# xh92117/Retinex-image-Enhancement

Hardware: AMD Instinct MI355X
Metric: images/sec at 512x512 bs=32 per GPU (UP-Retinex forward) (higher is better)
Workload: dtype f32; 1 GPU; configs[1]: bs=32/GPU 512x512 plain forward, fp32; global_batch=32, image_size=512, variant=plain, parallelism=batch-shard x1 (no data-path collective)

## Files before the change

include/upr.h:

```cpp
#ifndef UPR_H_
#define UPR_H_

#include <stddef.h>
#include <stdint.h>

#ifdef __cplusplus
extern "C" {
#endif

enum { UPR_F32 = 0, UPR_F16 = 1, UPR_F32_SPLIT = 2, UPR_F32_SPLIT_REGS = 3 };

enum {
  UPR_OK = 0,
  UPR_ERR_ARG = -1,
  UPR_ERR_SHAPE = -2,
  UPR_ERR_MISSING_PARAM = -3,
  UPR_ERR_WORKSPACE = -4,
  UPR_ERR_UNSUPPORTED = -5
};

enum { UPR_MODEL_IENET_ONLY = 1, UPR_MODEL_HEAD_ONLY = 2 };

typedef struct UprModel UprModel;

// ... 43 lines not shown
int upr_retinex_decompose_bwd(const void* x, const void* illu, const void* g, void* gx, void* gillu, int B, int C,
                              int H, int W, int illu_c, int dtype, void* stream);

int upr_conv2d_nhwc(const void* x, int B, int H, int W, int Cin, const void* w, const float* bias, int Cout, int kh,
                    int kw, int stride, int pad, int dil, const void* residual, int relu, void* y, int dtype,
                    void* stream);

int upr_conv2d_nhwc_regs(const void* x, int B, int H, int W, int Cin, const void* w, const float* bias, int Cout,
                         int kh, int kw, int stride, int pad, int dil, const void* residual, int relu, void* y,
                         unsigned* overflow, void* stream);

int upr_split_f32(const float* x, void* y, size_t npix, int C, unsigned* overflow, void* stream);
int upr_unsplit_f32(const void* x, float* y, size_t npix, int C, void* stream);
size_t upr_pack_split_f32(const float* w, int Cout, int Cin, int kh, int kw, void* out, size_t out_bytes);

size_t upr_pack_split_w_f32(const float* w, int Cout, int Cin, int kh, int kw, const float* w2, int C2, void* out,
                            size_t out_bytes);
int upr_conv2d_nhwc_wsplit(const void* x, int B, int H, int W, int Cin, const void* blob, size_t blob_bytes,
                           const float* bias, int Cout, int kh, int kw, int stride, int pad, int dil,
                           const void* residual, int relu, void* y, const void* x2, int H2, int W2, int C2,
                           int stride2, unsigned* overflow, void* stream);
int upr_conv_wsplit_ran(void);

int upr_quantize_u8(const void* x, uint8_t* out, size_t n, int dtype, void* stream);

int upr_letterbox(const void* src, int src_kind, int H, int W, int top, int left, int nh, int nw, int Ho, int Wo,
                  const int32_t* xtab, const int32_t* ytab, int color, void* out, int out_kind, void* stream);

int upr_to_u8_hwc(const void* x, int C, int H, int W, int dtype, uint8_t* out, void* stream);

int upr_rgb2lab_u8(const uint8_t* rgb, uint8_t* lab, size_t npix, void* stream);
int upr_lab2rgb_u8(const uint8_t* lab, uint8_t* rgb, size_t npix, void* stream);

int upr_clahe_u8(const uint8_t* src, uint8_t* dst, uint8_t* lut_ws, int B, int H, int W, float clip, int tiles_x,
                 int tiles_y, void* stream);

size_t upr_clahe_enhance_workspace(int B, int H, int W, int tiles_x, int tiles_y);
int upr_clahe_enhance(const void* enh, void* out, void* workspace, int B, int H, int W, float clip, int tiles_x,
                      int tiles_y, int dtype, void* stream);

int upr_gray_hist(const void* x, int32_t* hist, int B, int H, int W, int dtype, void* stream);

int upr_multiscale(const void* x, const void* enh, void* out, double* sums, double* factor, int B, int H, int W,
                   int dtype, void* stream);

int upr_multiscale_features(const void* x, void* out, int B, int H, int W, int scale_idx, int dtype, void* stream);
// ... 51 lines not shown
```

retinex-image-enhancement_amd/csrc/conv_t2.hip:

```cpp
#include <algorithm>
#include <cstdlib>
#include <cstring>

#include "upr_common.h"

namespace upr {

typedef _Float16 t2h8 __attribute__((ext_vector_type(8)));
typedef _Float16 t2h4 __attribute__((ext_vector_type(4)));
typedef float t2f4 __attribute__((ext_vector_type(4)));

template <int KC, int COUT>
struct ConvT2Cfg {
  static constexpr int N = 4 * COUT;
  static constexpr int NSPLIT = N / 128;
  static constexpr int KS = KC / 32;
  static constexpr int NT = 8;
  static constexpr int TEAMS = 4 / NSPLIT;
  static constexpr int QPW = COUT >= 128 ? 1 : 128 / COUT;
  static constexpr int ROWS = QPW >= 2 ? QPW / 2 : 1;
  static constexpr int XS = QPW >= 2 ? 32 : 16;
  static constexpr int RSTR = COUT + 8;
  static constexpr int LDSW = ROWS * XS * RSTR * 2;
  static constexpr int OCC = KC >= 256 ? 1 : 2;
// ... 153 lines not shown
    __builtin_amdgcn_fence(__ATOMIC_RELEASE, "wavefront");
    __builtin_amdgcn_wave_barrier();
    __builtin_amdgcn_fence(__ATOMIC_ACQUIRE, "wavefront");
    const int b = g / (H * gpr), rem = g - b * H * gpr, y = rem / gpr, xg = (rem - y * gpr) * 16;
    const int q0 = ns * K::QPW, dy0 = q0 >> 1;
    constexpr int CPP = COUT / 4;
    constexpr int CHUNKS = K::ROWS * K::XS * CPP;
#pragma unroll
    for (int i = 0; i < CHUNKS / 64; ++i) {
      const int c = i * 64 + lane;
      const int row = c / (K::XS * CPP), xs = (c / CPP) % K::XS, part = c % CPP;
      const int xo = K::QPW >= 2 ? 2 * xg + xs : 2 * (xg + xs) + (q0 & 1);
      const f4 v = *(const f4*)(st + ((row * K::XS + xs) * RSTR + part * 4) * 4);
      float* dst = (float*)op.out + ((size_t)(b * 2 * H + 2 * y + dy0 + row) * (2 * W) + xo) * op.out_cs +
                   op.out_coff + part * 4;
      *(f4*)dst = v;
    }
    __builtin_amdgcn_wave_barrier();
#pragma unroll
    for (int q = 0; q < KQ; ++q) x0[q] = x1[q];
  }
}

template <int KC, int COUT>
static int launch_t2_f32(const ConvOp& op, hipStream_t st) {
  static int occ = 0;
  if (!occ) {
    if (hipOccupancyMaxActiveBlocksPerMultiprocessor(&occ, (const void*)conv_t2_f32_kernel<KC, COUT>, 256, 0) !=
            hipSuccess ||
        occ < 1)
      occ = 1;
  }
  int cus = 256;
  {
    int dev = 0;
    if (hipGetDevice(&dev) == hipSuccess) (void)hipDeviceGetAttribute(&cus, hipDeviceAttributeMultiprocessorCount, dev);
  }
  const int ngroups = op.B * op.Ho * (op.Wo / 16);
  const int teams = ConvT2Cfg<KC, COUT>::TEAMS;
  int grid = std::min(cus * occ, (ngroups + teams - 1) / teams);
  if (grid < 1) grid = 1;
  hipLaunchKernelGGL((conv_t2_f32_kernel<KC, COUT>), dim3(grid), dim3(256), 0, st, op, ngroups);
  return (int)hipGetLastError();
}

template <int KC, int COUT>
// ... 44 lines not shown
```

retinex-image-enhancement_amd/csrc/model.hip:

```cpp
#include <algorithm>
#include <atomic>
#include <cmath>
#include <cstdio>
#include <cstdlib>
#include <cstring>
#include <map>
#include <memory>
#include <mutex>
#include <string>
#include <vector>

#include "upr_common.h"
#include "../../include/upr.h"

namespace upr {

int launch_prep(const void* x, void* x2p, void* x3p, int B, int H, int W, int dtype, hipStream_t st);
int launch_preact_f16(const void* x, const float* sc, const float* sh, void* o, size_t npix, int C, hipStream_t st);
int launch_conv3(const void* x, const float* w, const float* bias, void* out0, void* out1, int B, int h, int wd,
                 int dtype, hipStream_t st, void* out2 = nullptr, const float* ps = nullptr,
                 const float* ph = nullptr);
int launch_fam_ca(const float* pool, const float* w1, const float* b1, const float* w2, const float* b2, float* ca,
                  int B, int HW, hipStream_t st);
int launch_fam_mix(const void* y, const float* ca, const float* P, float* mm, float* p, int B, int HW, int dtype,
// ... 202 lines not shown
static bool pack_split_w(int N, int K, const float* w, SplitWPack& out) {
  if (!w || N <= 0 || N % 64 || K <= 0 || K % 32) return false;
  out.W.assign((size_t)N * K * 2, (_Float16)0.f);
  out.scale.assign(N, 1.f);
  for (int n = 0; n < N; ++n) {
    const float* row = w + (size_t)n * K;
    float mx = 0.f;
    for (int k = 0; k < K; ++k) mx = std::max(mx, std::fabs(row[k]));
    const int sh = split_row_shift(mx);
    const float s = std::ldexp(1.f, sh);
    out.scale[n] = std::ldexp(1.f, -sh);
    _Float16* dst = out.W.data() + (size_t)n * K * 2;
    for (int k = 0; k < K; ++k) {
      const float ws = row[k] * s;
      const _Float16 hi = (_Float16)ws;
      _Float16* step = dst + (size_t)(k / 32) * 64;
      step[wsplit_kslot(k % 32)] = hi;
      step[32 + wsplit_kslot(k % 32)] = (_Float16)(ws - (float)hi);
    }
  }
  return true;
}

static std::vector<double> conv_w(const HostTensor& t, const std::vector<double>* mul) {
  std::vector<double> w = t.v;
  if (mul) {
    const size_t per = w.size() / mul->size();
    for (size_t n = 0; n < mul->size(); ++n)
      for (size_t i = 0; i < per; ++i) w[n * per + i] *= (*mul)[n];
  }
  return w;
}

static std::vector<double> compose(const std::vector<double>& A, int O, int Mdim, const std::vector<double>& W,
                                   int C, int khw) {
  std::vector<double> out((size_t)O * C * khw, 0.0);
  for (int o = 0; o < O; ++o)
    for (int m = 0; m < Mdim; ++m) {
      const double a = A[(size_t)o * Mdim + m];
      if (a == 0.0) continue;
      for (int i = 0; i < C * khw; ++i) out[(size_t)o * C * khw + i] += a * W[(size_t)m * C * khw + i];
    }
  return out;
}

static std::vector<double> cols(const std::vector<double>& A, int rows, int ncols, int c0, int n) {
// ... 30 lines not shown
};

static std::vector<double> conv3_kmajor(const std::vector<double>& w) {
  const size_t nout = w.size() / 27;
  std::vector<double> t(w.size());
  for (size_t o = 0; o < nout; ++o)
    for (size_t k = 0; k < 27; ++k) t[k * nout + o] = w[o * 27 + k];
  return t;
}

enum OpKind { OP_GEMM, OP_CONV3, OP_PREP, OP_FAM_CA, OP_FAM_MIX, OP_FAM_SA, OP_ASPP_G, OP_TAIL, OP_PREACT, OP_SPLIT };

struct Op {
  OpKind kind;
  std::string name;
  int layer = -1;
  int level = 0;
  int out = -1, out_cs = 0, out_coff = 0;
  int res1 = -1, res1_cs = 0, res2 = -1, res2_cs = 0;
  int relu = 0, store = kStoreNHWC;
  int pool_slot = -1;
  int split_layer = -1, split_exit = 0;
  size_t w64_w = SIZE_MAX, w64_scale = 0;
  int img_bias = 0;
  size_t head_w = 0; float head_b = 0.f;
  int in = -1, out1 = -1, out2 = -1;
  size_t ps = 0, ph = 0;
  size_t w = 0, b = 0;
  int fam = 0;
  size_t ca_w1 = 0, ca_b1 = 0, ca_w2 = 0, ca_b2 = 0, P = 0, sa_w = 0;
  float sa_b = 0.f;
  int lvl_shift = 0;
  size_t cst = 0;
};

}

struct UprModel {
  int dtype = 0;
  int use_preact = 0, use_aspp = 0, flags = 0;
  void* dev_blob = nullptr;
  size_t blob_bytes = 0;
  std::vector<upr::GemmLayer> layers;
  std::vector<upr::Op> ops;
  bool prof = false;
  std::vector<std::vector<hipEvent_t>> ev_pending;
// ... 5 lines not shown
  struct Side {
    hipStream_t s = nullptr;
    hipEvent_t fork = nullptr, join = nullptr;
    unsigned long long last_use = 0;
    ~Side() {
      if (s) (void)hipStreamSynchronize(s);
      if (join) (void)hipEventDestroy(join);
      if (fork) (void)hipEventDestroy(fork);
      if (s) (void)hipStreamDestroy(s);
    }
  };
  static constexpr size_t kMaxSides = 16;
  std::map<std::pair<int, hipStream_t>, std::shared_ptr<Side>> sides;
  unsigned long long side_clock = 0;
  std::mutex sides_mu;
  std::atomic<long long> forks{0};
  std::atomic<int> split_state{0};
  unsigned* ovf_dev = nullptr;
  volatile unsigned* ovf_host = nullptr;
  int split_regs = 0;
  int ring_split = 0;
  int split_w64 = 0;
  int w64_tile = 0;
  std::vector<int> op_forms;
  std::mutex forms_mu;
};

namespace upr {

struct BufGeom {
  int C;
  int shift;
  int is_f32;
  int pyramid;
};

static BufGeom buf_geom(int id, int use_aspp) {
  switch (id) {
    case B_X2P: return {3, 2, 0, 1};
    case B_X3P: return {3, 4, 0, 2};
    case B_X1: case B_S1IN: return {32, 0, 0, 0};
    case B_S2IN: return {32, 2, 0, 1};
    case B_S3IN: return {32, 4, 0, 2};
    case B_E1T: case B_X2: return {64, 1, 0, 0};
    case B_E2T: case B_X3: return {128, 2, 0, 0};
    case B_E3T: case B_X4: case B_B0T: case B_B0: case B_AP: case B_B1T: case B_X5: return {256, 3, 0, 0};
// ... 102 lines not shown
      o->split_layer = (int)m->layers.size() - 1;
      o->split_exit = i + 1 == names.size();
    }
    return true;
  }
  void make_w64(const std::vector<std::string>& names) {
    if (dt != kF32) return;
    for (const std::string& name : names)
      for (auto& o : m->ops) {
        if (o.kind != OP_GEMM || o.name != name) continue;
        const GemmLayer& L = m->layers[o.layer];
        bool fits = L.N % 64 == 0 && o.store == kStoreNHWC && o.pool_slot < 0 && !o.img_bias && o.out2 < 0 &&
                    !L.segs.empty() && L.segs.size() <= 2;
        int K = 0;
        for (const SegSpec& s : L.segs) {
          fits = fits && s.pre == kPreNone && s.C % 32 == 0 && s.kbase == K;
          K += s.kh * s.kw * s.C;
        }
        SplitWPack sp;
        if (!fits || K != L.Kpad || !pack_split_w(L.N, K, (const float*)(blob.bytes.data() + L.w), sp)) continue;
        o.w64_w = blob.add(sp.W.data(), sp.W.size() * 2);
        o.w64_scale = blob.add(sp.scale.data(), sp.scale.size() * 4);
      }
  }
  void gemm(const std::string& name, int layer, int level, int out, int out_cs, int relu, int res1 = -1,
            int res1_cs = 0, int res2 = -1, int res2_cs = 0, int store = kStoreNHWC, int out_coff = 0,
            int pool_slot = -1, int img_bias = 0) {
    Op o;
    o.kind = OP_GEMM; o.name = name; o.layer = layer; o.level = level; o.out = out; o.out_cs = out_cs; o.out_coff = out_coff;
    o.relu = relu; o.res1 = res1; o.res1_cs = res1_cs; o.res2 = res2; o.res2_cs = res2_cs; o.store = store;
    o.pool_slot = pool_slot; o.img_bias = img_bias;
    m->ops.push_back(o);
  }

  void block(const std::string& p, int in, int tmp, int out, int cin, int cout, int stride, int in_level,
             int pool_slot = -1) {
    const int lvl = in_level + (stride == 2 ? 1 : 0);
    const bool proj = stride != 1 || cin != cout;
    const HostTensor* w1 = T(p + ".conv1.weight");
    const HostTensor* w2 = T(p + ".conv2.weight");
    if (!ok) return;
    if (!m->use_preact) {
      BNFold bn1, bn2, bns;
      if (!bn_fold(P, p + ".bn1", cout, bn1) || !bn_fold(P, p + ".bn2", cout, bn2)) { ok = false; return; }
      std::vector<SegWeights> s1(1);
      s1[0].spec = seg(in, cin, cin, 0, 3, stride, 1, 1);
// ... 260 lines not shown
    bd.block(ie + ".bottleneck.0", B_X4, B_B0T, B_B0, 256, 256, 1, 3, 3);
    bd.aspp(ie + ".bottleneck.1", B_B0, B_AP);
    bd.block(ie + ".bottleneck.2", B_AP, B_B1T, B_X5, 256, 256, 1, 3);
  } else {
    bd.block(ie + ".bottleneck.0", B_X4, B_B0T, B_B0, 256, 256, 1, 3);
    bd.block(ie + ".bottleneck.1", B_B0, B_B1T, B_X5, 256, 256, 1, 3);
  }
  if (!bd.ok) return P.missing.empty() ? kErrShape : kErrMissingParam;
  bd.upblock(ie + ".dec3", B_X5, B_U3, B_V3, B_D3, 256, 128, 3, B_X3);
  if (m->split_state.load() == 1) {
    std::vector<std::string> region;
    for (const char* n : {".enc2.conv1", ".enc2.conv2", ".enc3.conv1", ".enc3.conv2", ".bottleneck.0.conv1",
                          ".bottleneck.0.conv2", ".bottleneck.1.conv1", ".bottleneck.1.conv2", ".dec3.up",
                          ".dec3.conv.0", ".dec3.conv.3"})
      region.push_back(ie + n);
    if (!bd.ok || !bd.make_split(region)) {
      for (auto& o : m->ops) o.split_layer = -1;
      m->split_state.store(0);
    }
    bd.kept.clear();
  }
  bd.upblock(ie + ".dec2", B_D3, B_U2, B_V2, B_D2, 128, 64, 2, B_X2);
  bd.upblock(ie + ".dec1", B_D2, B_U1, B_V1, B_D1, 64, 32, 1, B_X1);
  if (bd.ok && m->split_state.load() == 1 && m->split_regs && m->split_w64)
    bd.make_w64({ie + ".enc1.conv1", ie + ".enc1.conv2", ie + ".dec2.conv.0", ie + ".dec2.conv.3"});
  {
    const HostTensor* w0 = bd.T(ie + ".residual_head.0.weight");
    const HostTensor* b0 = bd.T(ie + ".residual_head.0.bias");
    const HostTensor* w2 = bd.T(ie + ".residual_head.2.weight");
    const HostTensor* b2 = bd.T(ie + ".residual_head.2.bias");
    if (!bd.ok) return kErrMissingParam;
    std::vector<SegWeights> s(1);
    s[0].spec = seg(B_D1, 32, 32, 0, 3, 1, 1, 1);
    s[0].w = w0->v;
    int l = bd.add_layer(32, s, b0->v);
    Op o;
    o.kind = OP_GEMM; o.name = ie + ".residual_head"; o.layer = l; o.level = 0; o.store = kStoreHeadIllu;
    o.head_w = blob.add_f32(w2->v); o.head_b = (float)b2->v[0];
    m->ops.push_back(o);
  }
  }
  if (!(m->flags & UPR_MODEL_IENET_ONLY)) {
    const HostTensor* wfu = bd.T("fusion.weight");
    const HostTensor* bfu = bd.T("fusion.bias");
    const HostTensor* wo = bd.T("output_layer.weight");
    const HostTensor* bo = bd.T("output_layer.bias");
// ... 86 lines not shown
  float* pool = (float*)buf(B_POOL);
  float* ca = (float*)buf(B_CA);
  float* ib = (float*)buf(B_IB);
  UPR_CHECK_HIP(hipMemsetAsync(pool, 0, (size_t)4 * B * 256 * 4 * kPoolEntryFloats, st));
  const int H4 = (H / 2) / 2, W4 = (W / 2) / 2, H16 = (H / 4) / 4, W16 = (W / 4) / 4;
  auto lvl_dims = [&](int lshift, int& h, int& w) {
    if (lshift == 2) { h = H4; w = W4; }
    else if (lshift == 4) { h = H16; w = W16; }
    else { h = H >> lshift; w = W >> lshift; }
  };
  float* illu32 = dt == kF16 ? (float*)buf(B_ILLU32) : (float*)illu;
  const size_t nops = m->ops.size();
  std::vector<hipEvent_t> evs;
  if (m->prof) {
    evs.resize(2 * nops);
    for (auto& e : evs) {
      if (!m->ev_free.empty()) { e = m->ev_free.back(); m->ev_free.pop_back(); }
      else UPR_CHECK_HIP(hipEventCreate(&e));
    }
    m->cur_flops.assign(nops, 0.0);
    m->cur_bytes.assign(nops, 0.0);
  }
  const double elt = dt == kF16 ? 2.0 : 4.0;
  auto split_op = [&](const Op& o, int ho, int wo) {
    const GemmLayer& L = m->layers[o.split_layer];
    ConvOp c;
    memset(&c, 0, sizeof(c));
    c.nseg = (int)L.segs.size();
    for (int i = 0; i < c.nseg; ++i) {
      const SegSpec& s = L.segs[i];
      ConvSeg& cs = c.seg[i];
      cs.src = buf(s.src);
      cs.C = s.C; cs.cs = s.cs; cs.coff = s.coff;
      cs.Hin = ho * s.stride; cs.Win = wo * s.stride;
      cs.kh = s.kh; cs.kw = s.kw; cs.stride = s.stride; cs.pad = s.pad; cs.dil = s.dil;
      cs.pre = kPreNone; cs.kbase = s.kbase;
    }
    c.B = B; c.Ho = ho; c.Wo = wo; c.N = L.N; c.Kpad = L.Kpad;
    c.W = blob + L.w;
    c.scale = fptr(L.scale);
    c.bias = L.bias != SIZE_MAX ? fptr(L.bias) : nullptr;
    c.res1 = o.res1 >= 0 ? buf(o.res1) : nullptr; c.res1_cs = 2 * o.res1_cs;
    c.res2 = o.res2 >= 0 ? buf(o.res2) : nullptr; c.res2_cs = 2 * o.res2_cs;
    c.split_res = c.res1 || c.res2;
    c.relu = o.relu;
    c.store = o.store;
    if (o.split_exit) { c.out_f32 = (float*)buf(o.out); c.out_f32_cs = o.out_cs; }
    else { c.split_out = buf(o.out); c.split_cs = 2 * o.out_cs; c.split_lo = o.out_cs; }
    c.ovf = m->ovf_dev;
    return c;
  };
  bool split_now = false;
  if (m->split_state.load() == 1) {
    int one = 1;
    if (m->ovf_host && *m->ovf_host) {
      if (m->split_state.compare_exchange_strong(one, 2))
        fprintf(stderr, "upr: an fp32 activation left the fp16 range; this model now runs its exact fp32 plan "
                      "(UPR_FP32_SPLIT=0 selects it from the start)\n");
    } else {
      split_now = true;
      for (const Op& o : m->ops)
        if (o.kind == OP_GEMM && o.split_layer >= 0) {
          int ho, wo;
          lvl_dims(o.level, ho, wo);
          if (launch_conv_wide(split_op(o, ho, wo), st, true) != kOk) split_now = false;
        }
    }
  }
  const bool regs_now = m->split_regs && m->ovf_dev && m->split_state.load() == 1 && !(m->ovf_host && *m->ovf_host);
  std::vector<int> forms(nops, 0);
  auto run_op = [&](size_t oi, hipStream_t st) -> int {
    const Op& o = m->ops[oi];
    int rc = kOk;
    if (m->prof) UPR_CHECK_HIP(hipEventRecord(evs[2 * oi], st));
    switch (o.kind) {
      case OP_PREP:
        rc = launch_prep(x, buf(B_X2P), buf(B_X3P), B, H, W, dt, st);
        break;
      case OP_CONV3: {
        int h, w;
        lvl_dims(o.lvl_shift, h, w);
        rc = launch_conv3(buf(o.in), fptr(o.w), fptr(o.b), buf(o.out), o.out1 >= 0 ? buf(o.out1) : nullptr, B, h, w,
                          dt, st, o.out2 >= 0 ? buf(o.out2) : nullptr, o.out2 >= 0 ? fptr(o.ps) : nullptr,
                          o.out2 >= 0 ? fptr(o.ph) : nullptr);
        break;
      }
      case OP_GEMM: {
        const GemmLayer& L = m->layers[o.layer];
        ConvOp c;
// ... 16 lines not shown
        }
        c.B = B; c.Ho = ho; c.Wo = wo; c.N = L.N; c.Kpad = L.Kpad;
        c.W = blob + L.w;
        c.scale = nullptr;
        c.bias = L.bias != SIZE_MAX ? fptr(L.bias) : nullptr;
        c.img_bias = o.img_bias ? ib : nullptr;
        c.res1 = o.res1 >= 0 ? buf(o.res1) : nullptr; c.res1_cs = o.res1_cs;
        c.relu = o.relu;
        c.res2 = o.res2 >= 0 ? buf(o.res2) : nullptr; c.res2_cs = o.res2_cs;
        c.store = o.store;
        if (o.store == kStoreHeadIllu) {
          c.head_w = fptr(o.head_w); c.head_b = o.head_b;
          c.x_nchw = (const float*)x; c.x_f16 = dt == kF16;
          c.illu = illu32; c.illu_f16 = 0;
          c.out = nullptr;
        } else {
          c.out = buf(o.out); c.out_cs = o.out_cs; c.out_coff = o.out_coff;
        }
        c.pool = o.pool_slot >= 0 ? pool + (size_t)o.pool_slot * B * 256 * kPoolEntryFloats : nullptr;
        if (o.out2 >= 0) {
          c.out2 = buf(o.out2); c.out2_cs = L.N;
          c.pre2_scale = fptr(o.ps); c.pre2_shift = fptr(o.ph);
        }
        if (split_now && o.split_layer >= 0) {
          rc = launch_conv_wide(split_op(o, ho, wo), st);
          forms[oi] = 1;
        } else {
          rc = kErrUnsupported;
          if (regs_now && dt == kF32 && o.w64_w != SIZE_MAX) {
            ConvOp cw = c;
            cw.W = blob + o.w64_w; cw.scale = fptr(o.w64_scale);
            cw.mma16 = 3; cw.ovf = m->ovf_dev;
            cw.ring_split = m->ring_split; cw.w64_tile = m->w64_tile;
            rc = launch_conv_wsplit(cw, st);
            if (rc == kOk) forms[oi] = 3;
          }
          if (rc == kErrUnsupported) {
            if (regs_now && dt == kF32) { c.mma16 = 1; c.ovf = m->ovf_dev; c.ring_split = m->ring_split; }
            rc = launch_conv(c, dt, st);
            forms[oi] = conv_last_form();
          }
        }
        if (m->prof) {
          const double Mpx = (double)B * ho * wo;
          double K = 0, bytes = (double)L.N * L.Kpad * elt;
          for (int i = 0; i < c.nseg; ++i) {
            K += (double)c.seg[i].kh * c.seg[i].kw * c.seg[i].C;
            bytes += (double)B * c.seg[i].Hin * c.seg[i].Win * c.seg[i].C * elt;
          }
          const double nout = o.store == kStoreHeadIllu ? 1.0 : (double)L.N;
// ... 210 lines not shown
  if ((flags & ~kKnownFlags) || (flags & kKnownFlags) == kKnownFlags) return UPR_ERR_ARG;
  ParamSet P;
  for (int i = 0; i < n_params; ++i) {
    const UprTensorDesc& d = params[i];
    if (!d.name || d.ndim < 0 || d.ndim > 4) return UPR_ERR_ARG;
    HostTensor t;
    int64_t n = 1;
    for (int k = 0; k < d.ndim; ++k) { t.shape.push_back(d.shape[k]); n *= d.shape[k]; }
    if (n > 0 && !d.data) return UPR_ERR_ARG;
    t.v.assign(d.data, d.data + n);
    P.t[d.name] = std::move(t);
  }
  std::unique_ptr<UprModel> m(new UprModel());
  m->dtype = dtype; m->use_preact = use_preact ? 1 : 0; m->use_aspp = use_aspp ? 1 : 0; m->flags = flags;
  const char* se = getenv("UPR_FP32_SPLIT");
  const bool split_env = !(se && *se && atoi(se) == 0);
  if (split_env && dtype == UPR_F32 && !m->use_preact && !m->use_aspp) m->split_state.store(1);
  const char* sr = getenv("UPR_FP32_SPLIT_REGS");
  m->split_regs = !(sr && *sr && atoi(sr) == 0);
  m->ring_split = ring_split_env();
  const char* sw = getenv("UPR_FP32_SPLIT_W64");
  m->split_w64 = !(sw && *sw && atoi(sw) == 0);
  m->w64_tile = w64_tile_env();
  int rc = build_model(m.get(), P);
  if (rc == kOk && m->split_state.load() == 1) {
    hipError_t e = hipMalloc((void**)&m->ovf_dev, 256);
    if (e == hipSuccess) e = hipMemset(m->ovf_dev, 0, 256);
    if (e == hipSuccess) e = hipHostMalloc((void**)&m->ovf_host, sizeof(unsigned), hipHostMallocDefault);
    if (e == hipSuccess) *m->ovf_host = 0u;
    else rc = (int)e;
  }
  if (rc != kOk) {
    if (m->dev_blob) (void)hipFree(m->dev_blob);
    if (m->ovf_dev) (void)hipFree(m->ovf_dev);
    if (m->ovf_host) (void)hipHostFree((void*)m->ovf_host);
    return rc;
  }
  *out = m.release();
  return UPR_OK;
}

size_t upr_model_workspace(const UprModel* model, int B, int H, int W) {
  if (!model || B <= 0 || H <= 0 || W <= 0) return 0;
  return ws_layout(model, B, H, W, nullptr);
}

// ... 226 lines not shown
  memset(&c, 0, sizeof(c));
  c.nseg = x2 ? 2 : 1;
  ConvSeg& s = c.seg[0];
  s.src = x; s.C = Cin; s.cs = Cin; s.coff = 0; s.Hin = H; s.Win = W;
  s.kh = kh; s.kw = kw; s.stride = stride; s.pad = pad; s.dil = dil; s.pre = kPreNone; s.kbase = 0;
  if (x2) {
    ConvSeg& t = c.seg[1];
    t.src = x2; t.C = C2; t.cs = C2; t.coff = 0; t.Hin = H2; t.Win = W2;
    t.kh = 1; t.kw = 1; t.stride = stride2; t.pad = 0; t.dil = 1; t.pre = kPreNone; t.kbase = K1;
  }
  c.B = B; c.Ho = Ho; c.Wo = Wo; c.N = Cout; c.Kpad = K;
  c.W = blob; c.scale = (const float*)((const uint8_t*)blob + soff);
  c.bias = bias; c.relu = relu;
  c.res2 = residual; c.res2_cs = Cout;
  c.out = y; c.out_cs = Cout; c.out_coff = 0; c.store = kStoreNHWC;
  c.mma16 = 3; c.ovf = overflow;
  c.ring_split = ring_split_env();
  c.w64_tile = w64_tile_env();
  return launch_conv_wsplit(c, (hipStream_t)stream);
}

int upr_conv_wsplit_ran(void) { return conv_last_wsplit_kernel(); }

int upr_split_f32(const float* x, void* y, size_t npix, int C, unsigned* overflow, void* stream) {
  if (!x || !y) return UPR_ERR_ARG;
  return launch_split_f32(x, y, npix, C, overflow, (hipStream_t)stream);
}

int upr_unsplit_f32(const void* x, float* y, size_t npix, int C, void* stream) {
  if (!x || !y) return UPR_ERR_ARG;
  return launch_unsplit_f32(x, y, npix, C, (hipStream_t)stream);
}

}
```

retinex-image-enhancement_amd/csrc/upr_common.h:

```cpp
#pragma once
#include <hip/hip_runtime.h>
#include <stdint.h>
#include <stddef.h>

#define UPR_CHECK_HIP(expr)                                  \
  do {                                                       \
    hipError_t _e = (expr);                                  \
    if (_e != hipSuccess) return (int)_e;                    \
  } while (0)

namespace upr {

typedef _Float16 half_t;

enum : int {
  kOk = 0,
  kErrArg = -1,
  kErrShape = -2,
  kErrMissingParam = -3,
  kErrWorkspace = -4,
  kErrUnsupported = -5,
};

enum DType : int { kF32 = 0, kF16 = 1 };
// ... 94 lines not shown
  return sh;
}

int launch_split_f32(const float* x, void* y, size_t npix, int C, unsigned* ovf, hipStream_t st);
int launch_unsplit_f32(const void* x, float* y, size_t npix, int C, hipStream_t st);

int launch_conv_out32(const ConvOp& op, hipStream_t stream);
int launch_conv_s2dg(const ConvOp& op, hipStream_t stream, bool probe = false);
int launch_conv_pw(const ConvOp& op, hipStream_t stream, bool probe = false);

int launch_conv(const ConvOp& op, int dtype, hipStream_t stream);
int conv_last_form();
void conv_set_last_form(int form);
int launch_conv_regs(const ConvOp& op, hipStream_t stream);

int launch_conv_ring32(const ConvOp& op, hipStream_t st);
int launch_conv_wsplit(const ConvOp& op, hipStream_t st);
int launch_conv_ring_w64(const ConvOp& op, hipStream_t st);
int conv_last_wsplit_kernel();
void conv_reset_wsplit_kernel();
inline int wsplit_kslot(int c) { return ((c & 15) >> 2) * 8 + (c >> 4) * 4 + (c & 3); }
int launch_conv_wide(const ConvOp& op, hipStream_t st, bool probe = false);

inline int cdiv(int a, int b) { return (a + b - 1) / b; }

constexpr float kPoolScale = 16777216.f;
constexpr int kPoolEntryFloats = 4;
#ifdef __HIPCC__
__device__ __forceinline__ void pool_add(float* pool, size_t idx, float v) {
  if (__builtin_isfinite(v)) {
    atomicAdd((unsigned long long*)pool + 2 * idx, (unsigned long long)__float2ll_rn(v * kPoolScale));
  } else {
    const unsigned f = __builtin_isnan(v) ? 4u : (v > 0.f ? 1u : 2u);
    atomicOr((unsigned*)pool + 4 * idx + 2, f);
  }
}
__device__ __forceinline__ float pool_get(const float* pool, size_t idx) {
  const unsigned f = ((const unsigned*)pool)[4 * idx + 2];
  if (f) return (f & 4u) || (f & 3u) == 3u ? __builtin_nanf("") : ((f & 1u) ? __builtin_inff() : -__builtin_inff());
  return (float)((double)(long long)((const unsigned long long*)pool)[2 * idx] * (1.0 / 16777216.0));
}
#endif
inline size_t align_up(size_t v, size_t a) { return (v + a - 1) / a * a; }

constexpr int kScratchStreams = 64;
enum ScratchSlot { kSlotSlab = 0, kSlotCast, kSlotTmp, kSlotCode, kSlotRows, kSlotPart, kSlotMs, kSlotCount };
// ... 4 lines not shown
```

retinex-image-enhancement_amd/upr/_lib.py:

```python
import ctypes
import os

_HERE = os.path.dirname(os.path.abspath(__file__))
LIB_PATH = os.environ.get("UPR_LIB", os.path.join(os.path.dirname(_HERE), "lib", "libupr.so"))

UPR_F32 = 0
UPR_F16 = 1
UPR_F32_SPLIT = 2
UPR_F32_SPLIT_REGS = 3
UPR_MODEL_IENET_ONLY = 1
UPR_MODEL_HEAD_ONLY = 2

UPR_OK = 0
UPR_ERR_ARG = -1
UPR_ERR_SHAPE = -2
UPR_ERR_MISSING_PARAM = -3
UPR_ERR_WORKSPACE = -4
UPR_ERR_UNSUPPORTED = -5


class UprTensorDesc(ctypes.Structure):
    _fields_ = [("name", ctypes.c_char_p),
                ("data", ctypes.POINTER(ctypes.c_float)),
                ("ndim", ctypes.c_int),
# ... 35 lines not shown
                                 ctypes.POINTER(c_void_p)]),
    "upr_model_workspace": (c_size_t, [c_void_p, c_int, c_int, c_int]),
    "upr_model_forward": (c_int, [c_void_p, c_void_p, c_int, c_int, c_int, c_void_p, c_void_p, c_void_p,
                                  c_void_p, c_size_t, c_void_p]),
    "upr_model_destroy": (None, [c_void_p]),
    "upr_model_forks": (ctypes.c_longlong, [c_void_p]),
    "upr_model_split_state": (c_int, [c_void_p]),
    "upr_model_op_forms": (c_int, [c_void_p, ctypes.POINTER(UprOpForm), c_int]),
    "upr_model_profile": (c_int, [c_void_p, c_int]),
    "upr_model_profile_read": (c_int, [c_void_p, ctypes.POINTER(UprOpStat), c_int, ctypes.POINTER(c_int)]),
    "upr_status_string": (ctypes.c_char_p, [c_int]),
    "upr_conv2d_nhwc": (c_int, [c_void_p, c_int, c_int, c_int, c_int, c_void_p, c_void_p, c_int, c_int, c_int,
                                c_int, c_int, c_int, c_void_p, c_int, c_void_p, c_int, c_void_p]),
    "upr_conv2d_nhwc_regs": (c_int, [c_void_p, c_int, c_int, c_int, c_int, c_void_p, c_void_p, c_int, c_int, c_int,
                                     c_int, c_int, c_int, c_void_p, c_int, c_void_p, c_void_p, c_void_p]),
    "upr_split_f32": (c_int, [c_void_p, c_void_p, c_size_t, c_int, c_void_p, c_void_p]),
    "upr_unsplit_f32": (c_int, [c_void_p, c_void_p, c_size_t, c_int, c_void_p]),
    "upr_pack_split_f32": (c_size_t, [c_void_p, c_int, c_int, c_int, c_int, c_void_p, c_size_t]),
    "upr_pack_split_w_f32": (c_size_t, [c_void_p, c_int, c_int, c_int, c_int, c_void_p, c_int, c_void_p, c_size_t]),
    "upr_conv_wsplit_ran": (c_int, []),
    "upr_conv2d_nhwc_wsplit": (c_int, [c_void_p, c_int, c_int, c_int, c_int, c_void_p, c_size_t, c_void_p, c_int, c_int,
                                       c_int, c_int, c_int, c_int, c_void_p, c_int, c_void_p, c_void_p, c_int, c_int,
                                       c_int, c_int, c_void_p, c_void_p]),
    "upr_quantize_u8": (c_int, [c_void_p, c_void_p, c_size_t, c_int, c_void_p]),
    "upr_letterbox": (c_int, [c_void_p, c_int, c_int, c_int, c_int, c_int, c_int, c_int, c_int, c_int, c_void_p,
                              c_void_p, c_int, c_void_p, c_int, c_void_p]),
    "upr_to_u8_hwc": (c_int, [c_void_p, c_int, c_int, c_int, c_int, c_void_p, c_void_p]),
    "upr_rgb2lab_u8": (c_int, [c_void_p, c_void_p, c_size_t, c_void_p]),
    "upr_lab2rgb_u8": (c_int, [c_void_p, c_void_p, c_size_t, c_void_p]),
    "upr_clahe_u8": (c_int, [c_void_p, c_void_p, c_void_p, c_int, c_int, c_int, c_float, c_int, c_int, c_void_p]),
    "upr_clahe_enhance_workspace": (c_size_t, [c_int, c_int, c_int, c_int, c_int]),
    "upr_clahe_enhance": (c_int, [c_void_p, c_void_p, c_void_p, c_int, c_int, c_int, c_float, c_int, c_int, c_int,
                                  c_void_p]),
    "upr_gray_hist": (c_int, [c_void_p, c_void_p, c_int, c_int, c_int, c_int, c_void_p]),
    "upr_multiscale": (c_int, [c_void_p, c_void_p, c_void_p, c_void_p, c_void_p, c_int, c_int, c_int, c_int,
                               c_void_p]),
    "upr_multiscale_features": (c_int, [c_void_p, c_void_p, c_int, c_int, c_int, c_int, c_int, c_void_p]),
    "upr_content_aware_workspace": (c_size_t, [c_int, c_int, c_int]),
    "upr_content_aware": (c_int, [c_void_p, c_void_p, c_void_p, c_void_p, c_void_p, c_void_p, c_size_t, c_int, c_int,
                                  c_int, c_int, c_void_p]),
    "upr_image_metrics_workspace": (c_size_t, [c_int, c_int, c_int]),
    "upr_image_metrics": (c_int, [c_void_p, c_void_p, c_void_p, c_void_p, c_void_p, c_void_p, c_size_t, c_int, c_int,
                                  c_int, c_int, c_void_p]),
    "upr_png_bound": (c_int, [c_int, c_int, c_int, ctypes.POINTER(c_size_t), ctypes.POINTER(c_size_t)]),
    "upr_png_encode": (c_int, [c_void_p, c_int, c_int, c_int, c_int, c_int, c_void_p, c_size_t, c_void_p, c_void_p,
                               c_size_t, c_void_p]),
# ... 197 lines not shown
```

retinex-image-enhancement_amd/upr/runtime.py:

```python
import ctypes

import torch

from . import _lib as L

_DT = {torch.float32: L.UPR_F32, torch.float16: L.UPR_F16}


def dtype_code(dt):
    if dt not in _DT:
        raise TypeError(f"UP-Retinex HIP path supports float32 and float16 tensors, got {dt}")
    return _DT[dt]


def _require_device(t, name="input"):
    if not isinstance(t, torch.Tensor):
        raise TypeError(f"{name} must be a torch.Tensor")
    if t.device.type != "cuda":
        raise RuntimeError(
            f"{name} is on '{t.device}': the UP-Retinex framework executes on ROCm devices only "
            f"(MI355X HIP kernels); move the model and the tensor to a 'cuda' (ROCm) device")


def _ptr(t):
# ... 305 lines not shown
    x = x.contiguous()
    B, H, W, Cin = x.shape
    Ho = (H + 2 * pad - dil * (kh - 1) - 1) // stride + 1
    Wo = (W + 2 * pad - dil * (kw - 1) - 1) // stride + 1
    y = torch.empty((B, Ho, Wo, cout), dtype=x.dtype, device=x.device)
    if residual is not None:
        residual = residual.contiguous()
    H2 = W2 = C2 = 0
    if x2 is not None:
        x2 = x2.contiguous()
        _, H2, W2, C2 = x2.shape
    with torch.cuda.device(x.device):
        rc = L.lib().upr_conv2d_nhwc_wsplit(_ptr(x), B, H, W, Cin, _ptr(w_blob), w_blob.numel(), _ptr(bias), cout, kh,
                                            kw, stride, pad, dil, _ptr(residual), int(bool(relu)), _ptr(y), _ptr(x2),
                                            H2, W2, C2, stride2, _ptr(overflow), _stream(x.device))
    L.check(rc, "upr_conv2d_nhwc_wsplit")
    return y


def last_wsplit_kernel():
    return {1: "tile", 2: "ring"}.get(L.lib().upr_conv_wsplit_ran())


def split_f32(x, overflow=None):
    _require_device(x)
    if x.dtype != torch.float32 or x.shape[-1] % 8:
        raise ValueError("split_f32 expects float32 with a channel count that is a multiple of 8")
    x = x.contiguous()
    C = x.shape[-1]
    y = torch.empty(x.shape[:-1] + (2 * C,), dtype=torch.float16, device=x.device)
    with torch.cuda.device(x.device):
        rc = L.lib().upr_split_f32(_ptr(x), _ptr(y), x.numel() // C, C, _ptr(overflow), _stream(x.device))
    L.check(rc, "upr_split_f32")
    return y


def unsplit_f32(y):
    _require_device(y)
    if y.dtype != torch.float16 or y.shape[-1] % 16:
        raise ValueError("unsplit_f32 expects a float16 split tensor")
    y = y.contiguous()
    C = y.shape[-1] // 2
    x = torch.empty(y.shape[:-1] + (C,), dtype=torch.float32, device=y.device)
    with torch.cuda.device(y.device):
        rc = L.lib().upr_unsplit_f32(_ptr(y), _ptr(x), y.numel() // (2 * C), C, _stream(y.device))
    L.check(rc, "upr_unsplit_f32")
# ... 144 lines not shown
```

Before: 2444 images/s.

## Add split-fp16 MFMA kernel for 2x2 transposed convs fed by split exit

Adds a conv-transpose-2x2 kernel that emulates fp32 with hi/lo fp16 MFMA products using per-row scaled split weights. It can read the split fp16 tensor directly from the preceding split-exit layer, so that layer no longer has to write an fp32 output for the upsample. The intent is to replace the slower exact fp32 transposed conv in dec2.up (and optionally dec1.up) and drop a conversion pass. It is enabled by default through UPR_REGION_BORDERS, and dropping the lo*lo term carries a small accuracy risk.

```diff
diff --git a/include/upr.h b/include/upr.h
--- a/include/upr.h
+++ b/include/upr.h
@@ -89,6 +89,11 @@
                            int stride2, unsigned* overflow, void* stream);
 int upr_conv_wsplit_ran(void);
 
+size_t upr_pack_split_t2_f32(const float* w, int Cout, int Cin, void* out, size_t out_bytes);
+int upr_conv_transpose2x2_nhwc(const void* x, int B, int H, int W, int Cin, const void* w, size_t w_bytes,
+                               const float* bias, int Cout, int relu, int form, float* y, unsigned* overflow,
+                               void* stream);
+
 int upr_quantize_u8(const void* x, uint8_t* out, size_t n, int dtype, void* stream);
 
 int upr_letterbox(const void* src, int src_kind, int H, int W, int top, int left, int nh, int nw, int Ho, int Wo,
diff --git a/retinex-image-enhancement_amd/csrc/conv_t2.hip b/retinex-image-enhancement_amd/csrc/conv_t2.hip
--- a/retinex-image-enhancement_amd/csrc/conv_t2.hip
+++ b/retinex-image-enhancement_amd/csrc/conv_t2.hip
@@ -199,6 +199,166 @@
   }
 }
 
+template <int KC, int COUT, int SRC_SPLIT>
+__global__ __launch_bounds__(256, (KC >= 128 ? 1 : 2)) void conv_t2_f32_kernel_split(ConvOp op, int ngroups) {
+  using K = ConvT2Cfg<KC, COUT>;
+  constexpr int RSTR = COUT + 4;
+  constexpr int LDSW = K::ROWS * K::XS * RSTR * 4;
+  typedef float f4 __attribute__((ext_vector_type(4)));
+  __shared__ __attribute__((aligned(16))) unsigned char stage[4 * LDSW];
+  __shared__ __attribute__((aligned(16))) float bs[2 * K::N];
+  const int tid = threadIdx.x, lane = tid & 63;
+  const int wave = __builtin_amdgcn_readfirstlane(tid >> 6);
+  const int fr = lane & 15, fg = lane >> 4;
+  const int ns = wave % K::NSPLIT, team = wave / K::NSPLIT;
+  unsigned char* st = stage + wave * LDSW;
+  const ConvSeg& sg = op.seg[0];
+  const int cs = sg.cs;
+  const int H = op.Ho, W = op.Wo, gpr = W / 16;
+
+  for (int i = tid; i < K::N; i += 256) {
+    bs[i] = op.bias ? op.bias[i] : 0.f;
+    bs[K::N + i] = op.scale[i];
+  }
+  t2h8 wh[K::NT][K::KS], wl[K::NT][K::KS];
+#pragma unroll
+  for (int nt = 0; nt < K::NT; ++nt)
+#pragma unroll
+    for (int ks = 0; ks < K::KS; ++ks) {
+      const size_t f = (((size_t)(ns * K::NT + nt) * K::KS + ks) * 64 + lane) * 8;
+      wh[nt][ks] = *(const t2h8*)((const half_t*)op.W + f);
+      wl[nt][ks] = *(const t2h8*)((const half_t*)op.W + (size_t)K::N * KC + f);
+    }
+  __syncthreads();
+
+  const int stride = gridDim.x * K::TEAMS;
+  int g = blockIdx.x * K::TEAMS + team;
+  struct Px {
+    t2h8 hi[K::KS], lo[K::KS];
+    f4 v[2 * K::KS];
+  };
+  auto load = [&](int gg, Px& x) {
+    if (gg < ngroups) {
+      if (SRC_SPLIT) {
+        const half_t* p = (const half_t*)sg.src + sg.coff + ((size_t)gg * 16 + fr) * cs + fg * 8;
+#pragma unroll
+        for (int ks = 0; ks < K::KS; ++ks) {
+          x.hi[ks] = *(const t2h8*)(p + ks * 32);
+          x.lo[ks] = *(const t2h8*)(p + KC + ks * 32);
+        }
+      } else {
+        const float* p = (const float*)sg.src + sg.coff + ((size_t)gg * 16 + fr) * cs + fg * 8;
+#pragma unroll
+        for (int ks = 0; ks < K::KS; ++ks) {
+          x.v[2 * ks] = *(const f4*)(p + ks * 32);
+          x.v[2 * ks + 1] = *(const f4*)(p + ks * 32 + 4);
+        }
+      }
+    }
+  };
+  constexpr bool DEEP = KC >= 128;
+  Px x0, x1, x2;
+  load(g, x0);
+  if (DEEP) load(g + stride, x1);
+  bool bad = false;
+  for (; g < ngroups; g += stride) {
+    if (DEEP) load(g + 2 * stride, x2);
+    else load(g + stride, x1);
+    f4 acc[K::NT], acc2[K::NT];
+#pragma unroll
+    for (int nt = 0; nt < K::NT; ++nt) acc[nt] = acc2[nt] = f4{0.f, 0.f, 0.f, 0.f};
+#pragma unroll
+    for (int ks = 0; ks < K::KS; ++ks) {
+      t2h8 hi, lo;
+      if (SRC_SPLIT) {
+        hi = x0.hi[ks];
+        lo = x0.lo[ks];
+      } else {
+        const float v[8] = {x0.v[2 * ks][0],     x0.v[2 * ks][1],     x0.v[2 * ks][2],     x0.v[2 * ks][3],
+                            x0.v[2 * ks + 1][0], x0.v[2 * ks + 1][1], x0.v[2 * ks + 1][2], x0.v[2 * ks + 1][3]};
+        split_f32x8(v, hi, lo);
+      }
+#pragma unroll
+      for (int nt = 0; nt < K::NT; ++nt) {
+        acc[nt] = __builtin_amdgcn_mfma_f32_16x16x32_f16(wh[nt][ks], hi, acc[nt], 0, 0, 0);
+        acc2[nt] = __builtin_amdgcn_mfma_f32_16x16x32_f16(wh[nt][ks], lo, acc2[nt], 0, 0, 0);
+        acc[nt] = __builtin_amdgcn_mfma_f32_16x16x32_f16(wl[nt][ks], hi, acc[nt], 0, 0, 0);
+      }
+    }
+#pragma unroll
+    for (int nt = 0; nt < K::NT; ++nt) {
+      const int nl = nt * 16 + fg * 4;
+      const int ql = nl / COUT, co = nl % COUT;
+      const int row = ql >> 1, xs = K::QPW >= 2 ? 2 * fr + (ql & 1) : fr;
+      const f4 b = *(const f4*)(bs + ns * 128 + nl), sc = *(const f4*)(bs + K::N + ns * 128 + nl);
+      f4 o;
+#pragma unroll
+      for (int r = 0; r < 4; ++r) {
+        o[r] = __builtin_fmaf(__builtin_fmaf(acc2[nt][r], kSplitLoInv, acc[nt][r]), sc[r], b[r]);
+        if (!SRC_SPLIT) bad |= !(__builtin_fabsf(o[r]) <= 3.4028234664e38f);
+        if (op.relu) o[r] = fmaxf(o[r], 0.f);
+      }
+      *(f4*)(st + ((row * K::XS + xs) * RSTR + co) * 4) = o;
+    }
+    __builtin_amdgcn_fence(__ATOMIC_RELEASE, "wavefront");
+    __builtin_amdgcn_wave_barrier();
+    __builtin_amdgcn_fence(__ATOMIC_ACQUIRE, "wavefront");
+    const int b = g / (H * gpr), rem = g - b * H * gpr, y = rem / gpr, xg = (rem - y * gpr) * 16;
+    const int q0 = ns * K::QPW, dy0 = q0 >> 1;
+    constexpr int CPP = COUT / 4;
+    constexpr int CHUNKS = K::ROWS * K::XS * CPP;
+#pragma unroll
+    for (int i = 0; i < CHUNKS / 64; ++i) {
+      const int c = i * 64 + lane;
+      const int row = c / (K::XS * CPP), xs = (c / CPP) % K::XS, part = c % CPP;
+      const int xo = K::QPW >= 2 ? 2 * xg + xs : 2 * (xg + xs) + (q0 & 1);
+      const f4 v = *(const f4*)(st + ((row * K::XS + xs) * RSTR + part * 4) * 4);
+      float* dst = (float*)op.out + ((size_t)(b * 2 * H + 2 * y + dy0 + row) * (2 * W) + xo) * op.out_cs +
+                   op.out_coff + part * 4;
+      *(f4*)dst = v;
+    }
+    __builtin_amdgcn_wave_barrier();
+    x0 = x1;
+    if (DEEP) x1 = x2;
+  }
+  if (!SRC_SPLIT && bad && op.ovf) *op.ovf = 1u;
+}
+
+template <int KC, int COUT, int SRC_SPLIT>
+static int launch_t2_split(const ConvOp& op, hipStream_t st) {
+  int cus = 256;
+  {
+    int dev = 0;
+    if (hipGetDevice(&dev) == hipSuccess) (void)hipDeviceGetAttribute(&cus, hipDeviceAttributeMultiprocessorCount, dev);
+  }
+  const int ngroups = op.B * op.Ho * (op.Wo / 16);
+  const int teams = ConvT2Cfg<KC, COUT>::TEAMS;
+  int grid = std::min(cus * (KC >= 128 ? 1 : 2), (ngroups + teams - 1) / teams);
+  if (grid < 1) grid = 1;
+  hipLaunchKernelGGL((conv_t2_f32_kernel_split<KC, COUT, SRC_SPLIT>), dim3(grid), dim3(256), 0, st, op, ngroups);
+  return (int)hipGetLastError();
+}
+
+int launch_conv_t2_split(const ConvOp& op, int src_split, hipStream_t st, bool probe) {
+  if (op.store != kStoreConvT2x2 || op.nseg != 1 || !op.W || !op.scale || !op.out) return kErrUnsupported;
+  if (op.res1 || op.res2 || op.pool || op.img_bias || op.out2 || op.out32 || op.split_out || op.out_f32)
+    return kErrUnsupported;
+  const ConvSeg& s = op.seg[0];
+  if (s.kh != 1 || s.kw != 1 || s.stride != 1 || s.pad != 0 || s.pre != kPreNone || s.kbase != 0) return kErrUnsupported;
+  if (s.Hin != op.Ho || s.Win != op.Wo || op.Wo % 16 || op.B <= 0 || op.Ho <= 0 || (uintptr_t)s.src % 16)
+    return kErrUnsupported;
+  if (src_split ? (s.cs % 8 || s.coff % 8 || s.cs < s.coff + 2 * s.C) : (s.cs % 4 || s.coff % 4 || s.cs < s.coff + s.C))
+    return kErrUnsupported;
+  if (op.out_cs % 4 || op.out_coff % 4 || op.out_cs < op.out_coff + op.N / 4 || (uintptr_t)op.out % 16 ||
+      (uintptr_t)op.W % 16 || op.Kpad != s.C)
+    return kErrUnsupported;
+  if ((long long)op.B * op.Ho * op.Wo > (1LL << 31) / 32) return kErrUnsupported;
+  const bool k128 = s.C == 128 && op.N == 256 && src_split, k64 = s.C == 64 && op.N == 128 && !src_split;
+  if (!k128 && !k64) return kErrUnsupported;
+  if (probe) return kOk;
+  return k128 ? launch_t2_split<128, 64, 1>(op, st) : launch_t2_split<64, 32, 0>(op, st);
+}
+
 template <int KC, int COUT>
 static int launch_t2_f32(const ConvOp& op, hipStream_t st) {
   static int occ = 0;
diff --git a/retinex-image-enhancement_amd/csrc/model.hip b/retinex-image-enhancement_amd/csrc/model.hip
--- a/retinex-image-enhancement_amd/csrc/model.hip
+++ b/retinex-image-enhancement_amd/csrc/model.hip
@@ -248,6 +248,32 @@
   return true;
 }
 
+static bool pack_split_t2(int N, int K, const double* w, SplitWPack& out) {
+  if (!w || N <= 0 || N % 128 || K <= 0 || K % 32) return false;
+  const size_t plane = (size_t)N * K;
+  out.W.assign(2 * plane, (_Float16)0.f);
+  out.scale.assign(N, 1.f);
+  for (int n = 0; n < N; ++n) {
+    const double* row = w + (size_t)n * K;
+    double mx = 0.0;
+    for (int k = 0; k < K; ++k) mx = std::max(mx, std::fabs(row[k]));
+    int e = 15;
+    if (mx > 0.0 && std::isfinite(mx)) (void)std::frexp(mx, &e);
+    const int sh = std::min(std::max(15 - e, -100), 100);
+    const double sc = std::ldexp(1.0, sh);
+    out.scale[n] = (float)std::ldexp(1.0, -sh);
+    for (int k = 0; k < K; ++k) {
+      const double ws = row[k] * sc;
+      const _Float16 hi = (_Float16)ws;
+      const int lane = ((k % 32) / 8) * 16 + n % 16;
+      const size_t f = (((size_t)(n / 16) * (K / 32) + k / 32) * 64 + lane) * 8 + k % 8;
+      out.W[f] = hi;
+      out.W[plane + f] = (_Float16)(ws - (double)hi);
+    }
+  }
+  return true;
+}
+
 static std::vector<double> conv_w(const HostTensor& t, const std::vector<double>* mul) {
   std::vector<double> w = t.v;
   if (mul) {
@@ -324,6 +350,8 @@
   int pool_slot = -1;
   int split_layer = -1, split_exit = 0;
   size_t w64_w = SIZE_MAX, w64_scale = 0;
+  size_t t2_w = SIZE_MAX, t2_scale = 0;
+  int t2_src_split = 0;
   int img_bias = 0;
   size_t head_w = 0; float head_b = 0.f;
   int in = -1, out1 = -1, out2 = -1;
@@ -375,6 +403,7 @@
   int ring_split = 0;
   int split_w64 = 0;
   int w64_tile = 0;
+  int borders = 0, t2_regs = 0;
   std::vector<int> op_forms;
   std::mutex forms_mu;
 };
@@ -523,6 +552,20 @@
         o.w64_w = blob.add(sp.W.data(), sp.W.size() * 2);
         o.w64_scale = blob.add(sp.scale.data(), sp.scale.size() * 4);
       }
+  }
+  void make_t2(const std::string& name, int src_split) {
+    if (dt != kF32) return;
+    for (auto& o : m->ops) {
+      if (o.kind != OP_GEMM || o.name != name || o.store != kStoreConvT2x2 || !kept.count(o.layer)) continue;
+      const GemmLayer& L = m->layers[o.layer];
+      const std::vector<SegWeights>& sw = kept[o.layer];
+      if (sw.size() != 1 || sw[0].spec.kh != 1 || sw[0].spec.kw != 1 || sw[0].spec.C != L.Kpad) continue;
+      SplitWPack sp;
+      if (!pack_split_t2(L.N, L.Kpad, sw[0].w.data(), sp)) continue;
+      o.t2_w = blob.add(sp.W.data(), sp.W.size() * 2);
+      o.t2_scale = blob.add(sp.scale.data(), sp.scale.size() * 4);
+      o.t2_src_split = src_split;
+    }
   }
   void gemm(const std::string& name, int layer, int level, int out, int out_cs, int relu, int res1 = -1,
             int res1_cs = 0, int res2 = -1, int res2_cs = 0, int store = kStoreNHWC, int out_coff = 0,
@@ -829,6 +872,11 @@
   }
   bd.upblock(ie + ".dec2", B_D3, B_U2, B_V2, B_D2, 128, 64, 2, B_X2);
   bd.upblock(ie + ".dec1", B_D2, B_U1, B_V1, B_D1, 64, 32, 1, B_X1);
+  if (bd.ok && m->split_state.load() == 1 && m->borders) {
+    bd.make_t2(ie + ".dec2.up", 1);
+    if (m->t2_regs && m->split_regs) bd.make_t2(ie + ".dec1.up", 0);
+  }
+  bd.kept.clear();
   if (bd.ok && m->split_state.load() == 1 && m->split_regs && m->split_w64)
     bd.make_w64({ie + ".enc1.conv1", ie + ".enc1.conv2", ie + ".dec2.conv.0", ie + ".dec2.conv.3"});
   {
@@ -961,7 +1009,7 @@
     m->cur_bytes.assign(nops, 0.0);
   }
   const double elt = dt == kF16 ? 2.0 : 4.0;
-  auto split_op = [&](const Op& o, int ho, int wo) {
+  auto split_op = [&](const Op& o, int ho, int wo, bool exit_split = false) {
     const GemmLayer& L = m->layers[o.split_layer];
     ConvOp c;
     memset(&c, 0, sizeof(c));
@@ -984,7 +1032,7 @@
     c.split_res = c.res1 || c.res2;
     c.relu = o.relu;
     c.store = o.store;
-    if (o.split_exit) { c.out_f32 = (float*)buf(o.out); c.out_f32_cs = o.out_cs; }
+    if (o.split_exit && !exit_split) { c.out_f32 = (float*)buf(o.out); c.out_f32_cs = o.out_cs; }
     else { c.split_out = buf(o.out); c.split_cs = 2 * o.out_cs; c.split_lo = o.out_cs; }
     c.ovf = m->ovf_dev;
     return c;
@@ -1004,6 +1052,45 @@
           lvl_dims(o.level, ho, wo);
           if (launch_conv_wide(split_op(o, ho, wo), st, true) != kOk) split_now = false;
         }
+    }
+  }
+  auto t2_op = [&](const Op& o, int ho, int wo) {
+    const GemmLayer& L = m->layers[o.layer];
+    const SegSpec& s = L.segs[0];
+    ConvOp c;
+    memset(&c, 0, sizeof(c));
+    c.nseg = 1;
+    ConvSeg& cs = c.seg[0];
+    cs.src = buf(s.src);
+    cs.C = s.C; cs.cs = o.t2_src_split ? 2 * s.cs : s.cs; cs.coff = s.coff;
+    cs.Hin = ho; cs.Win = wo;
+    cs.kh = 1; cs.kw = 1; cs.stride = 1; cs.pad = 0; cs.dil = 1;
+    cs.pre = kPreNone; cs.kbase = 0;
+    c.B = B; c.Ho = ho; c.Wo = wo; c.N = L.N; c.Kpad = L.Kpad;
+    c.W = blob + o.t2_w;
+    c.scale = fptr(o.t2_scale);
+    c.bias = L.bias != SIZE_MAX ? fptr(L.bias) : nullptr;
+    c.relu = o.relu;
+    c.out = buf(o.out); c.out_cs = o.out_cs; c.out_coff = o.out_coff;
+    c.store = o.store;
+    c.ovf = m->ovf_dev;
+    return c;
+  };
+  bool exit_now = false;
+  if (split_now && m->borders) {
+    const Op* ex = nullptr;
+    const Op* up = nullptr;
+    for (const Op& o : m->ops) {
+      if (o.kind != OP_GEMM) continue;
+      if (o.split_layer >= 0 && o.split_exit) ex = &o;
+      if (o.t2_w != SIZE_MAX && o.t2_src_split) up = &o;
+    }
+    if (ex && up && m->layers[up->layer].segs.size() == 1 && m->layers[up->layer].segs[0].src == ex->out) {
+      int ho, wo;
+      lvl_dims(up->level, ho, wo);
+      exit_now = launch_conv_t2_split(t2_op(*up, ho, wo), 1, st, true) == kOk;
+      lvl_dims(ex->level, ho, wo);
+      if (exit_now && launch_conv_wide(split_op(*ex, ho, wo, true), st, true) != kOk) exit_now = false;
     }
   }
   const bool regs_now = m->split_regs && m->ovf_dev && m->split_state.load() == 1 && !(m->ovf_host && *m->ovf_host);
@@ -1066,10 +1153,15 @@
           c.out2 = buf(o.out2); c.out2_cs = L.N;
           c.pre2_scale = fptr(o.ps); c.pre2_shift = fptr(o.ph);
         }
+        const bool t2 = o.t2_w != SIZE_MAX && (o.t2_src_split ? exit_now : regs_now);
+        if (t2) {
+          rc = launch_conv_t2_split(t2_op(o, ho, wo), o.t2_src_split, st);
+          if (rc == kOk) forms[oi] = 4;
+        }
         if (split_now && o.split_layer >= 0) {
-          rc = launch_conv_wide(split_op(o, ho, wo), st);
+          rc = launch_conv_wide(split_op(o, ho, wo, exit_now), st);
           forms[oi] = 1;
-        } else {
+        } else if (!t2 || (rc == kErrUnsupported && !o.t2_src_split)) {
           rc = kErrUnsupported;
           if (regs_now && dt == kF32 && o.w64_w != SIZE_MAX) {
             ConvOp cw = c;
@@ -1326,6 +1418,9 @@
   const char* sw = getenv("UPR_FP32_SPLIT_W64");
   m->split_w64 = !(sw && *sw && atoi(sw) == 0);
   m->w64_tile = w64_tile_env();
+  const char* rb = getenv("UPR_REGION_BORDERS");
+  m->borders = !(rb && *rb && atoi(rb) == 0);
+  m->t2_regs = rb && *rb && atoi(rb) == 2;
   int rc = build_model(m.get(), P);
   if (rc == kOk && m->split_state.load() == 1) {
     hipError_t e = hipMalloc((void**)&m->ovf_dev, 256);
@@ -1598,6 +1693,49 @@
 
 int upr_conv_wsplit_ran(void) { return conv_last_wsplit_kernel(); }
 
+size_t upr_pack_split_t2_f32(const float* w, int Cout, int Cin, void* out, size_t out_bytes) {
+  if (!w || Cout <= 0 || Cout % 32 || Cin <= 0 || Cin % 32) return 0;
+  const int N = 4 * Cout;
+  std::vector<double> rows((size_t)N * Cin);
+  for (int q = 0; q < 4; ++q)
+    for (int co = 0; co < Cout; ++co)
+      for (int ci = 0; ci < Cin; ++ci)
+        rows[(size_t)(q * Cout + co) * Cin + ci] = w[(((size_t)ci * Cout + co) * 2 + (q >> 1)) * 2 + (q & 1)];
+  SplitWPack sp;
+  if (!pack_split_t2(N, Cin, rows.data(), sp)) return 0;
+  size_t soff = 0;
+  const size_t need = split_w_bytes(N, Cin, &soff);
+  if (out && out_bytes >= need) {
+    memset(out, 0, need);
+    memcpy(out, sp.W.data(), sp.W.size() * 2);
+    memcpy((uint8_t*)out + soff, sp.scale.data(), sp.scale.size() * 4);
+  }
+  return need;
+}
+
+int upr_conv_transpose2x2_nhwc(const void* x, int B, int H, int W, int Cin, const void* w, size_t w_bytes,
+                               const float* bias, int Cout, int relu, int form, float* y, unsigned* overflow,
+                               void* stream) {
+  if (!x || !w || !y || B <= 0 || H <= 0 || W <= 0 || Cin <= 0 || Cout <= 0 || form < 0 || form > 2) return UPR_ERR_ARG;
+  if (Cin % 32 || Cout % 32) return UPR_ERR_UNSUPPORTED;
+  const int N = 4 * Cout;
+  size_t soff = 0;
+  if (w_bytes != (form == 0 ? (size_t)N * Cin * 4 : split_w_bytes(N, Cin, &soff))) return UPR_ERR_UNSUPPORTED;
+  ConvOp c;
+  memset(&c, 0, sizeof(c));
+  c.nseg = 1;
+  ConvSeg& s = c.seg[0];
+  s.src = x; s.C = Cin; s.cs = form == 1 ? 2 * Cin : Cin; s.coff = 0; s.Hin = H; s.Win = W;
+  s.kh = 1; s.kw = 1; s.stride = 1; s.pad = 0; s.dil = 1; s.pre = kPreNone; s.kbase = 0;
+  c.B = B; c.Ho = H; c.Wo = W; c.N = N; c.Kpad = Cin;
+  c.W = w; c.bias = bias; c.relu = relu;
+  c.out = y; c.out_cs = Cout; c.out_coff = 0; c.store = kStoreConvT2x2;
+  if (form == 0) return launch_conv_t2(c, kF32, (hipStream_t)stream);
+  c.scale = (const float*)((const uint8_t*)w + soff);
+  c.ovf = overflow;
+  return launch_conv_t2_split(c, form == 1, (hipStream_t)stream);
+}
+
 int upr_split_f32(const float* x, void* y, size_t npix, int C, unsigned* overflow, void* stream) {
   if (!x || !y) return UPR_ERR_ARG;
   return launch_split_f32(x, y, npix, C, overflow, (hipStream_t)stream);
diff --git a/retinex-image-enhancement_amd/csrc/upr_common.h b/retinex-image-enhancement_amd/csrc/upr_common.h
--- a/retinex-image-enhancement_amd/csrc/upr_common.h
+++ b/retinex-image-enhancement_amd/csrc/upr_common.h
@@ -140,6 +140,9 @@
 inline int wsplit_kslot(int c) { return ((c & 15) >> 2) * 8 + (c >> 4) * 4 + (c & 3); }
 int launch_conv_wide(const ConvOp& op, hipStream_t st, bool probe = false);
 
+int launch_conv_t2(const ConvOp& op, int dtype, hipStream_t st);
+int launch_conv_t2_split(const ConvOp& op, int src_split, hipStream_t st, bool probe = false);
+
 inline int cdiv(int a, int b) { return (a + b - 1) / b; }
 
 constexpr float kPoolScale = 16777216.f;
diff --git a/retinex-image-enhancement_amd/upr/_lib.py b/retinex-image-enhancement_amd/upr/_lib.py
--- a/retinex-image-enhancement_amd/upr/_lib.py
+++ b/retinex-image-enhancement_amd/upr/_lib.py
@@ -81,6 +81,9 @@
     "upr_conv2d_nhwc_wsplit": (c_int, [c_void_p, c_int, c_int, c_int, c_int, c_void_p, c_size_t, c_void_p, c_int, c_int,
                                        c_int, c_int, c_int, c_int, c_void_p, c_int, c_void_p, c_void_p, c_int, c_int,
                                        c_int, c_int, c_void_p, c_void_p]),
+    "upr_pack_split_t2_f32": (c_size_t, [c_void_p, c_int, c_int, c_void_p, c_size_t]),
+    "upr_conv_transpose2x2_nhwc": (c_int, [c_void_p, c_int, c_int, c_int, c_int, c_void_p, c_size_t, c_void_p, c_int,
+                                           c_int, c_int, c_void_p, c_void_p, c_void_p]),
     "upr_quantize_u8": (c_int, [c_void_p, c_void_p, c_size_t, c_int, c_void_p]),
     "upr_letterbox": (c_int, [c_void_p, c_int, c_int, c_int, c_int, c_int, c_int, c_int, c_int, c_int, c_void_p,
                               c_void_p, c_int, c_void_p, c_int, c_void_p]),
diff --git a/retinex-image-enhancement_amd/upr/runtime.py b/retinex-image-enhancement_amd/upr/runtime.py
--- a/retinex-image-enhancement_amd/upr/runtime.py
+++ b/retinex-image-enhancement_amd/upr/runtime.py
@@ -351,6 +351,39 @@
     return {1: "tile", 2: "ring"}.get(L.lib().upr_conv_wsplit_ran())
 
 
+def pack_split_t2(w):
+    wc = w.detach().to("cpu", torch.float32).contiguous()
+    ci, co = wc.shape[:2]
+    lib = L.lib()
+    need = lib.upr_pack_split_t2_f32(ctypes.c_void_p(wc.data_ptr()), co, ci, None, 0) if wc.shape[2:] == (2, 2) else 0
+    if need == 0:
+        raise ValueError(f"pack_split_t2: unsupported weight shape {tuple(wc.shape)} ([Cin % 32, Cout % 32, 2, 2])")
+    blob = torch.empty(need, dtype=torch.uint8)
+    lib.upr_pack_split_t2_f32(ctypes.c_void_p(wc.data_ptr()), co, ci, ctypes.c_void_p(blob.data_ptr()), need)
+    return blob
+
+
+def conv_transpose2x2_nhwc(x, w, cout, bias=None, relu=False, form="exact", overflow=None):
+    _require_device(x)
+    code = {"exact": 0, "split": 1, "regs": 2}[form]
+    if x.dtype != (torch.float16 if code == 1 else torch.float32):
+        raise ValueError(f"conv_transpose2x2_nhwc form {form!r}: wrong input dtype {x.dtype}")
+    x = x.contiguous()
+    B, H, W, C = x.shape
+    cin = C // 2 if code == 1 else C
+    if code == 0:
+        w = w.to(torch.float32).permute(2, 3, 1, 0).reshape(4 * cout, cin).contiguous()
+    w = w.contiguous()
+    bias4 = None if bias is None else bias.to(torch.float32).repeat(4).contiguous()
+    y = torch.empty((B, 2 * H, 2 * W, cout), dtype=torch.float32, device=x.device)
+    with torch.cuda.device(x.device):
+        rc = L.lib().upr_conv_transpose2x2_nhwc(_ptr(x), B, H, W, cin, _ptr(w), w.numel() * w.element_size(),
+                                                _ptr(bias4), cout, int(bool(relu)), code, _ptr(y), _ptr(overflow),
+                                                _stream(x.device))
+    L.check(rc, "upr_conv_transpose2x2_nhwc")
+    return y
+
+
 def split_f32(x, overflow=None):
     _require_device(x)
     if x.dtype != torch.float32 or x.shape[-1] % 8:
```

Result: no change. 2458 images/s (median of 6 runs) (+0.6%).
